# pranoyr/attention-models

Measured on AMD Instinct MI355X. Metric: ViTVQGAN 256px train-step images/sec, higher is better.
Workload: dtype f32; 1 GPU; BASELINE.json configs[2]: ViTVQGAN dim=256 patch=8 img=256 depth=6+6 h=8 d=64 mlp=2048 (SwiGLU), codebook 8192x32; GAN train step (D phase + G phase, gradient penalty, per_loss_weight=0), Adam, clip 1.0; global_batch=32, batch_per_gpu=32, parallelism=dp1

## Files before the change

### attention-models_amd/amk/lib.py

```python
import ctypes
import os
import re

_HERE = os.path.dirname(os.path.abspath(__file__))
LIB_PATH = os.environ.get("AMK_LIB") or os.path.join(_HERE, "libamk.so")
HEADER_PATH = os.path.normpath(os.path.join(_HERE, "..", "..", "include", "amk.h"))

AMK_OK = 0

_c = ctypes
_P = _c.c_void_p
_I = _c.c_int
_L = _c.c_int64
_F = _c.c_float



class GemmDesc(_c.Structure):
    _fields_ = [("op", _c.c_int32), ("epilogue", _c.c_int32), ("m", _L),
                ("n", _c.c_int32), ("k", _c.c_int32), ("split", _c.c_int32), ("reserved", _c.c_int32),
                ("a", _P), ("a2", _P), ("w", _P), ("w2", _P), ("c", _P), ("c2", _P),
                ("lda", _L), ("lda2", _L), ("ldw", _L), ("ldw2", _L), ("ldc", _L), ("ldc2", _L),
                ("bias", _P), ("bias2", _P), ("resid", _P), ("ldr", _L),
                ("ln_mean", _P), ("ln_rstd", _P), ("ln_gamma", _P), ("ln_beta", _P),
                ("ab", _P), ("ldab", _L), ("gate", _P), ("ldg", _L), ("dbias", _P)]


GEMM_NT, GEMM_NN, GEMM_TN = 0, 1, 2
EPI_BIAS, EPI_RESID, EPI_SWIGLU, EPI_SWIGLU_BWD = 0, 1, 2, 3

SIGNATURES = {
    "amk_version": (_I, []),
    "amk_arch": (_c.c_char_p, []),
    "amk_last_error": (_c.c_char_p, []),
    "amk_attn_fwd": (_I, [_P] * 7 + [_I] * 5 + [_L] * 12 + [_F, _P]),
    "amk_attn_scores_bytes": (_L, [_I, _I, _I, _I]),
    "amk_attn_fwd_keep": (_I, [_P] * 8 + [_I] * 5 + [_L] * 12 + [_F, _P]),
    "amk_attn_fwd_x6_ws_bytes": (_L, [_I, _I, _I]),
    "amk_attn_fwd_x6": (_I, [_P] * 8 + [_I] * 5 + [_L] * 12 + [_F, _P]),
    "amk_attn_bwd_ws_floats": (_L, [_I, _I, _I, _I, _I]),
    "amk_attn_bwd": (_I, [_P] * 12 + [_I] * 5 + [_L] * 24 + [_F, _I, _P]),
    "amk_attn_bwd_kept": (_I, [_P] * 13 + [_I] * 5 + [_L] * 24 + [_F, _I, _P]),
    "amk_vq_num_partials": (_L, [_L]),
    "amk_vq_lookup_fwd": (_I, [_P, _P, _L, _I, _I, _I] + [_P] * 9 + [_P]),
    "amk_vq_lookup_bwd": (_I, [_P] * 7 + [_F, _L, _I, _I, _P, _P, _P]),
    "amk_vq_lookup_bwd_rows": (_I, [_P] * 7 + [_F, _L, _I, _I, _P, _P, _P]),
    "amk_vq_padded_codes": (_I, [_I, _I]),
    "amk_vq_gather": (_I, [_P, _P, _L, _I, _I, _P, _P, _P]),
    "amk_agent_num_chunks": (_I, [_I]),
    "amk_agent_ws_floats": (_L, [_I, _I, _I, _I, _I]),
    "amk_agent_attn_fwd": (_I, [_P] * 10 + [_I] * 5 + [_L] * 12 + [_F, _P]),
    "amk_agent_attn_bwd": (_I, [_P] * 14 + [_I] * 5 + [_L] * 21 + [_F, _P]),
    "amk_agent_conv_grad_reduce": (_I, [_P, _P, _L, _I, _P, _P, _P]),
    "amk_rowsum_num_partials": (_I, [_L]),
    "amk_add_layernorm_fwd": (_I, [_P, _P, _P, _P, _L, _I, _F, _P, _P, _P, _P, _P]),
    "amk_add_layernorm_bwd": (_I, [_P, _P, _P, _P, _P, _P, _L, _I, _P, _P, _P]),
    "amk_colsum": (_I, [_P, _L, _I, _P, _P]),
    "amk_swiglu_fwd": (_I, [_P, _L, _I, _P, _P]),
    "amk_swiglu_bwd": (_I, [_P, _P, _L, _I, _P, _P]),
    "amk_geglu_fwd": (_I, [_P, _L, _I, _P, _P]),
    "amk_geglu_bwd": (_I, [_P, _P, _L, _I, _P, _P]),
    "amk_opt_num_partials": (_I, []),
    "amk_sumsq_partials": (_I, [_P, _L, _P, _P]),
    "amk_adam_flat_step": (_I, [_P] * 4 + [_L, _P, _P, _P, _I] + [_F] * 6 + [_I, _P, _P]),
    "amk_adam_flat_step_shadow": (_I, [_P] * 4 + [_L, _P, _P, _P, _I] + [_F] * 6 + [_I, _P, _P, _P]),
    "amk_gemm_x6_planes_bytes": (_L, [_I, _I]),
    "amk_gemm_x6_split": (_I, [_P, _L, _I, _I, _P, _P]),
    "amk_gemm_x6_nt": (_I, [_P, _L, _P, _P, _P, _L, _I, _I, _I, _P]),
    "amk_gemm_f32_ws_bytes": (_L, [_c.POINTER(GemmDesc)]),
    "amk_gemm_f32": (_I, [_c.POINTER(GemmDesc), _P, _L, _P]),
    "amk_row_stats": (_I, [_P, _L, _I, _F, _P, _P, _P]),
    "amk_attn_bf16_fwd": (_I, [_P] * 7 + [_I] * 5 + [_L] * 12 + [_F, _P]),
    "amk_attn_bf16_bwd_ws_floats": (_L, [_I, _I, _I, _I]),
    "amk_attn_bf16_bwd": (_I, [_P] * 12 + [_I] * 5 + [_L] * 24 + [_F, _P]),
    "amk_swiglu_bf16_fwd": (_I, [_P, _L, _I, _P, _P]),
    "amk_swiglu_bf16_bwd": (_I, [_P, _P, _L, _I, _P, _P]),
    "amk_add_layernorm_mixed_fwd": (_I, [_P, _I, _P, _P, _P, _L, _I, _F, _P, _P, _P, _P, _P]),
    "amk_add_layernorm_mixed_bwd": (_I, [_P, _I, _P, _P, _P, _P, _P, _L, _I, _P, _P, _P, _P]),
    "amk_gemm_bf16": (_I, [_I, _I, _P, _L, _P, _L, _P, _P, _L, _P, _L, _L, _I, _I, _P]),
    "amk_gemm_bf16_swiglu_bwd": (_I, [_P, _L, _P, _L, _P, _L, _P, _L, _L, _I, _I, _P]),
    "amk_gemm_tn_bf16_ws_bytes": (_L, [_L, _I, _I]),
    "amk_gemm_tn_bf16": (_I, [_P, _L, _P, _L, _P, _L, _P, _L, _I, _I, _P, _L, _P]),
    "amk_sample_step": (_I, [_P, _P, _F, _P, _c.c_uint64, _c.c_uint64, _F, _L, _I, _I, _P, _F, _P, _P, _P]),
    "amk_moe_route_ws_ints": (_L, [_L, _I, _I]),
    "amk_moe_route": (_I, [_P, _L, _I, _I] + [_P] * 8),
    "amk_grouped_gemm_nt": (_I, [_P, _L, _I, _P, _P, _P, _P, _L, _I, _I, _I, _P, _P]),
    "amk_grouped_gemm_nn": (_I, [_P, _L, _I, _P, _P, _P, _P, _L, _I, _I, _I, _P, _P]),
    "amk_grouped_gemm_nt_acc": (_I, [_P, _L, _I, _P, _P, _P, _P, _L, _I, _I, _I, _P, _I, _P]),
    "amk_grouped_gemm_nn_acc": (_I, [_P, _L, _I, _P, _P, _P, _P, _L, _I, _I, _I, _P, _I, _P]),
    "amk_grouped_gemm_wgrad": (_I, [_P, _L, _I, _P, _L, _I, _P, _P, _P, _L, _I, _I, _I, _P, _P, _P]),
    "amk_moe_combine": (_I, [_P, _P, _P, _L, _I, _I, _I, _P, _P]),
    "amk_moe_expert_sums": (_I, [_P, _L, _I, _P, _P, _L, _I, _I, _I, _P, _P]),
    "amk_moe_topk": (_I, [_P, _L, _I, _I, _P, _P, _P]),
    "amk_moe_route_distinct": (_I, [_P, _L, _I, _I, _P, _P, _P, _P]),
    "amk_moe_combine_rows": (_I, [_P, _P, _P, _L, _I, _I, _I, _I, _I, _P, _P]),
    "amk_moe_gate_grad_rows": (_I, [_P, _P, _P, _P, _L, _I, _I, _I, _I, _I, _P, _P]),
    "amk_moe_gate_grad": (_I, [_P, _P, _P, _P, _L, _I, _I, _I, _I, _P, _P]),
}

_lib = None


def declared_symbols(header_path=HEADER_PATH):
    text = open(header_path).read()
    text = re.sub(r"/\*.*?\*/", "", text, flags=re.S)
    return sorted(set(re.findall(r"\b(amk_[a-z0-9_]+)\s*\(", text)))


def load():
    global _lib
    if _lib is not None:
        return _lib
    if not os.path.exists(LIB_PATH):
        raise RuntimeError(
            f"{LIB_PATH} is missing: build it with `python -c 'import __graft_entry__ as g; g.build()'` "
            "(hipcc --offload-arch=gfx950). amk has no CPU or eager fallback."
        )
    lib = ctypes.CDLL(LIB_PATH)
    for name, (res, args) in SIGNATURES.items():
        fn = getattr(lib, name)
        fn.restype = res
        fn.argtypes = args
    arch = lib.amk_arch().decode()
    if arch != "gfx950":
        raise RuntimeError(f"libamk.so was built for {arch}, expected gfx950")
    _lib = lib
    return lib


def check(rc, what):
    if rc != AMK_OK:
        msg = load().amk_last_error().decode()
        raise RuntimeError(f"{what} failed with code {rc}: {msg}")
```

### attention-models_amd/amk/models/discriminator.py

```python
import contextlib

import torch
import torch.nn as nn
import torch.nn.functional as F
from torch.nn.grad import conv2d_input, conv2d_weight

_INPUT_GRAD_ONLY = False


@contextlib.contextmanager
def input_grad_only():
    global _INPUT_GRAD_ONLY
    old, _INPUT_GRAD_ONLY = _INPUT_GRAD_ONLY, True
    try:
        yield
    finally:
        _INPUT_GRAD_ONLY = old


class _ConvDataGrad(torch.autograd.Function):

    @staticmethod
    def forward(ctx, gy, weight, x_shape, stride, padding):
        ctx.save_for_backward(gy, weight)
        ctx.cfg = (stride, padding)
        return conv2d_input(x_shape, weight, gy, stride=stride, padding=padding)

    @staticmethod
    def backward(ctx, ggx):
        gy, weight = ctx.saved_tensors
        stride, padding = ctx.cfg
        ggx = ggx.contiguous()
        ggy = F.conv2d(ggx, weight, None, stride, padding) if ctx.needs_input_grad[0] else None
        gw = conv2d_weight(ggx, weight.shape, gy, stride=stride, padding=padding) if ctx.needs_input_grad[1] else None
        return ggy, gw, None, None, None


class _Conv(torch.autograd.Function):
    @staticmethod
    def forward(ctx, x, weight, bias, stride, padding):
        ctx.save_for_backward(x, weight)
        ctx.cfg = (stride, padding, bias is not None)
        return F.conv2d(x, weight, bias, stride, padding)

    @staticmethod
    def backward(ctx, gy):
        x, weight = ctx.saved_tensors
        stride, padding, has_bias = ctx.cfg
        gy = gy.contiguous()
        gx = _ConvDataGrad.apply(gy, weight, x.shape, stride, padding) if ctx.needs_input_grad[0] else None
        gw = gb = None
        if not _INPUT_GRAD_ONLY:
            if ctx.needs_input_grad[1]:
                gw = conv2d_weight(x, weight.shape, gy, stride=stride, padding=padding)
            if has_bias and ctx.needs_input_grad[2]:
                gb = gy.sum((0, 2, 3))
        return gx, gw, gb, None, None


class Conv2d(nn.Conv2d):

    def forward(self, x):
        if self.groups != 1 or self.dilation != (1, 1) or self.padding_mode != "zeros" or isinstance(self.padding, str):
            return super().forward(x)
        if torch.is_autocast_enabled():
            if self.in_channels < 8 and x.is_cuda:
                with torch.autocast("cuda", enabled=False):
                    return _Conv.apply(x.float(), self.weight, self.bias, self.stride, self.padding)
            return super().forward(x)
        return _Conv.apply(x, self.weight, self.bias, self.stride, self.padding)


class NLayerDiscriminator(nn.Module):
    def __init__(self, input_nc=3, ndf=64, n_layers=3):
        super().__init__()
        widths = [ndf * min(2 ** i, 8) for i in range(n_layers + 1)]
        layers = [Conv2d(input_nc, widths[0], 4, stride=2, padding=1), nn.LeakyReLU(0.2, True)]
        for i in range(1, n_layers + 1):
            stride = 2 if i < n_layers else 1
            layers += [
                Conv2d(widths[i - 1], widths[i], 4, stride=stride, padding=1, bias=False),
                nn.BatchNorm2d(widths[i]),
                nn.LeakyReLU(0.2, True),
            ]
        layers.append(Conv2d(widths[-1], 1, 4, stride=1, padding=1))
        self.model = nn.Sequential(*layers)

    def forward(self, x):
        return self.model(x)
```

### attention-models_amd/amk/ops.py

```python
import ctypes
import os
import weakref

import torch
from torch.autograd.function import once_differentiable

from . import lib as _lib

_NULL = ctypes.c_void_p(0)


def _ptr(t):
    return ctypes.c_void_p(t.data_ptr()) if t is not None else _NULL


def _stream():
    return ctypes.c_void_p(torch.cuda.current_stream().cuda_stream)


KERNEL_EVENTS = None


class _timed:

# ... 1256 lines not shown
        dwa = dwb = None
        if ctx.needs_input_grad[1] or ctx.needs_input_grad[2]:
            (ar, av), (br, bv) = _claim(ctx.params[0]), _claim(ctx.params[1])
            dwa, dwb, _ = dense.gemm_tn(da2, x2, y2=db2, out=av, out2=bv)
            if av is not None:
                ar.wrote(ctx.params[0])
                dwa = None
            if bv is not None:
                br.wrote(ctx.params[1])
                dwb = None
        return dx, dwa, dwb


class _SwiGLUFFN(torch.autograd.Function):

    @staticmethod
    def forward(ctx, x, w12, b12, w3, b3):
        from . import dense

        x2 = x.reshape(-1, x.shape[-1])
        need = any(ctx.needs_input_grad)
        gate, ab = dense.gemm_nt_swiglu(x2, w12, b12, keep_ab=need)
        out = dense.gemm_nt(gate, w3, b3)
        if need:
            ctx.save_for_backward(x2, w12, w3, ab, gate)
        ctx.x_shape = x.shape
        ctx.has_bias = (b12 is not None, b3 is not None)
        ctx.params = (w12, b12, w3, b3)
        return out.view(*x.shape[:-1], w3.shape[0])

    @staticmethod
    @once_differentiable
    def backward(ctx, dout):
        from . import dense

        x2, w12, w3, ab, gate = ctx.saved_tensors
        d2 = dout.reshape(-1, dout.shape[-1])
        d_ab = dense.gemm_nn(d2, w3, swiglu_ab=ab)
        dw3, db3 = _tn_into(dense.gemm_tn, d2, gate, ctx.params[2], ctx.params[3] if ctx.has_bias[1] else None)
        dx = _nn_plain(d_ab, w12).view(ctx.x_shape) if ctx.needs_input_grad[0] else None
        dw12, db12 = _tn_into(dense.gemm_tn, d_ab, x2, ctx.params[0], ctx.params[1] if ctx.has_bias[0] else None)
        return dx, dw12, db12, dw3, db3


MIXED_WGRAD = os.environ.get("AMK_MIXED_WGRAD", "1") == "1"


def _w16(t):
    if t is None:
        return None
    shadow = getattr(t, "_amk_bf16", None)
    if shadow is not None and t._version == t._amk_bf16_version:
        return shadow
    return t.to(torch.bfloat16)


class _LinearMixed(torch.autograd.Function):

    @staticmethod
    def forward(ctx, x, weight, bias):
        x16, w16 = x.to(torch.bfloat16), _w16(weight)
        ctx.save_for_backward(x16, w16)
        ctx.has_bias, ctx.x_dtype = bias is not None, x.dtype
        ctx.params = (weight, bias)
        return torch.nn.functional.linear(x16, w16, _w16(bias))

    @staticmethod
    @once_differentiable
    def backward(ctx, dy):
        from . import dense

        x16, w16 = ctx.saved_tensors
        dy2 = dy.reshape(-1, dy.shape[-1])
        dx = dy2.mm(w16).view(x16.shape).to(ctx.x_dtype) if ctx.needs_input_grad[0] else None
        dw, db = _tn_into(dense.gemm_tn_bf16, dy2, x16.reshape(-1, x16.shape[-1]), ctx.params[0], ctx.params[1])
        return dx, dw, db


def _mixed_linear_ok(x, weight):
    return (MIXED_WGRAD and x.is_cuda and torch.get_autocast_dtype("cuda") == torch.bfloat16 and torch.is_grad_enabled()
            and weight.requires_grad and weight.dtype == torch.float32 and x.dtype in (torch.float32, torch.bfloat16)
            and weight.shape[0] % 8 == 0 and weight.shape[1] % 8 == 0 and x.numel() > 0)


def linear(x, weight, bias=None):
    if torch.is_autocast_enabled():
        if _mixed_linear_ok(x, weight):
            return _LinearMixed.apply(x, weight, bias)
        return torch.nn.functional.linear(x, weight, bias)
    if GEMM_MODE == "bf16x6" and _x6_ok(x, weight):
        return _LinearX6.apply(x, weight, bias)
    if _dense_ok(x, weight):
        return _DenseLinear.apply(x, weight, bias)
    if bias is None:
        return torch.nn.functional.linear(x, weight)
    return _BiasLinear.apply(x, weight, bias)


def linear2(x, wa, wb):
    if GEMM_MODE != "bf16x6" and _dense_ok(x, wa, wb) and wa.shape[0] % 128 == 0:
        return _DenseLinear2.apply(x, wa, wb)
    return linear(x, wa), linear(x, wb)


class _SwiGLUFFNMixed(torch.autograd.Function):

    @staticmethod
    def forward(ctx, x, w12, b12, w3, b3):
        from . import dense

        x16 = x.to(torch.bfloat16).reshape(-1, x.shape[-1])
        w12h, w3h = _w16(w12), _w16(w3)
        g, ab = dense.gemm_nt_swiglu_bf16(x16, w12h, b12)
        y = torch.nn.functional.linear(g, w3h, _w16(b3))
        ctx.save_for_backward(x16, ab, g, w12h, w3h)
        ctx.x_shape, ctx.x_dtype, ctx.bias = x.shape, x.dtype, (b12 is not None, b3 is not None)
        ctx.params = (w12, b12, w3, b3)
        return y.view(*x.shape[:-1], w3.shape[0])

    @staticmethod
    @once_differentiable
    def backward(ctx, dy):
        from . import dense

        x16, ab, g, w12h, w3h = ctx.saved_tensors
        dy2 = dy.reshape(-1, dy.shape[-1])
        dw3, db3 = _tn_into(dense.gemm_tn_bf16, dy2, g, ctx.params[2], ctx.params[3])
        dab = dense.gemm_nn_swiglu_bwd_bf16(dy2, w3h, ab)
        dw12, db12 = _tn_into(dense.gemm_tn_bf16, dab, x16, ctx.params[0], ctx.params[1])
        dx = dab.mm(w12h).view(ctx.x_shape).to(ctx.x_dtype) if ctx.needs_input_grad[0] else None
        return dx, dw12, db12, dw3, db3


def swiglu_ffn(x, w12, b12, w3, b3):
    if torch.is_autocast_enabled() and w12.shape[0] % 16 == 0 and w12.shape[0] >= 1024:
        if _mixed_linear_ok(x, w12) and _mixed_linear_ok(x, w3) and w3.requires_grad:
            with torch.autocast("cuda", enabled=False):
                return _SwiGLUFFNMixed.apply(x, w12, b12, w3, b3)
        no_grad = not torch.is_grad_enabled() or not any(
            t is not None and t.requires_grad for t in (x, w12, b12, w3, b3))
        if (MIXED_WGRAD and no_grad and x.is_cuda and torch.get_autocast_dtype("cuda") == torch.bfloat16
                and w12.dtype == torch.float32 and x.dtype in (torch.float32, torch.bfloat16) and w12.shape[1] % 8 == 0 and x.numel()):
            from . import dense

            g, _ = dense.gemm_nt_swiglu_bf16(x.to(torch.bfloat16).reshape(-1, x.shape[-1]), _w16(w12), b12, keep_ab=False)
            return torch.nn.functional.linear(g, _w16(w3), _w16(b3)).view(*x.shape[:-1], w3.shape[0])
    if GEMM_MODE != "bf16x6" and _dense_ok(x, w12) and w3.shape[1] % 4 == 0 and w3.shape[0] % 4 == 0 and w3.is_contiguous():
        return _SwiGLUFFN.apply(x, w12, b12, w3, b3)
    ab = linear(x, w12, b12)
    if ab.shape[-1] % 8 == 0:
        return linear(swiglu(ab), w3, b3)
    a, b = ab.chunk(2, dim=-1)
    return linear(torch.nn.functional.silu(a) * b, w3, b3)
```

### include/amk.h

```cpp
#ifndef AMK_H_
#define AMK_H_

#include <stdint.h>

#ifdef __cplusplus
extern "C" {
#endif

#define AMK_VERSION 140

enum {
  AMK_OK = 0,
  AMK_EINVAL = -1,
  AMK_EUNSUPPORTED = -2,
  AMK_ELAUNCH = -3
};

int amk_version(void);
const char* amk_arch(void);
const char* amk_last_error(void);

int amk_attn_fwd(const float* q, const float* k, const float* v, float* o, float* stats,
                 const uint8_t* key_mask, const uint8_t* causal_mask,
                 int B, int H, int I, int J, int D,
// ... 56 lines not shown
                      int64_t q_sb, int64_t q_st, int64_t q_sh,
                      int64_t k_sb, int64_t k_st, int64_t k_sh,
                      int64_t v_sb, int64_t v_st, int64_t v_sh,
                      int64_t o_sb, int64_t o_st, int64_t o_sh,
                      int64_t do_sb, int64_t do_st, int64_t do_sh,
                      int64_t dq_sb, int64_t dq_st, int64_t dq_sh,
                      int64_t dk_sb, int64_t dk_st, int64_t dk_sh,
                      int64_t dv_sb, int64_t dv_st, int64_t dv_sh,
                      float scale, int stages, void* stream);

int64_t amk_vq_num_partials(int64_t N);
int amk_vq_padded_codes(int K, int nsplit);
int amk_vq_lookup_fwd(const float* z, const float* codebook, int64_t N, int K, int C, int nsplit,
                      float* en_ws, float* ee_ws, float* pmin_ws, int32_t* pidx_ws,
                      int64_t* idx, float* out, float* zq, float* zn, float* sqerr_partial,
                      void* stream);

int amk_vq_lookup_bwd(const float* z, const float* codebook, const float* zn, const float* zq,
                      const int64_t* idx, const float* g_out, const float* g_loss, float beta,
                      int64_t N, int K, int C, float* dz, float* dcodebook, void* stream);

int amk_vq_lookup_bwd_rows(const float* z, const float* codebook, const float* zn, const float* zq,
                           const int64_t* idx, const float* g_out, const float* g_loss, float beta,
                           int64_t N, int K, int C, float* dz, float* ge_rows, void* stream);

int amk_vq_gather(const int64_t* idx, const float* codebook, int64_t N, int K, int C,
                  float* out, int32_t* bad_count, void* stream);


int64_t amk_moe_route_ws_ints(int64_t U, int E, int k);
int amk_moe_route(const float* logits, int64_t U, int E, int k,
                  int64_t* ids, float* gate, int32_t* counts, int32_t* rank, int32_t* blockhist,
                  int32_t* offsets, int32_t* perm, void* stream);

int amk_grouped_gemm_nt(const float* A, int64_t lda, int a_div, const float* W, const float* bias,
                        const int32_t* offsets, const int32_t* perm, int64_t P, int E, int N, int Kd,
                        float* Y, void* stream);

int amk_grouped_gemm_nn(const float* A, int64_t lda, int a_div, const float* W, const float* scale,
                        const int32_t* offsets, const int32_t* perm, int64_t P, int E, int N, int Kd,
                        float* Y, void* stream);

int amk_grouped_gemm_nt_acc(const float* A, int64_t lda, int a_div, const float* W, const float* bias,
                            const int32_t* offsets, const int32_t* perm, int64_t P, int E, int N, int Kd,
                            float* Y, int y_div, void* stream);
int amk_grouped_gemm_nn_acc(const float* A, int64_t lda, int a_div, const float* W, const float* scale,
                            const int32_t* offsets, const int32_t* perm, int64_t P, int E, int N, int Kd,
                            float* Y, int y_div, void* stream);

int amk_grouped_gemm_wgrad(const float* G, int64_t ldg, int g_div, const float* X, int64_t ldx, int x_div,
                           const float* scale, const int32_t* offsets, const int32_t* perm,
                           int64_t P, int E, int N, int Kd, float* dW, float* dbias, void* stream);

int amk_moe_combine(const float* Y, const int64_t* ids, const float* scale, int64_t G, int outer, int k,
                    int N, float* out, void* stream);

int amk_moe_topk(const float* logits, int64_t U, int E, int k, int64_t* ids, float* gate, void* stream);

int amk_moe_route_distinct(const int64_t* ids, int64_t G, int fan, int E, uint64_t* mask,
                           int32_t* offsets, int32_t* perm, void* stream);

int amk_moe_combine_rows(const float* Y, const int64_t* ids, const float* scale, int64_t G, int outer, int k,
                         int N, int v_div, int E, float* out, void* stream);
int amk_moe_gate_grad_rows(const float* d_out, const float* Y, const int64_t* ids, const float* gate,
                           int64_t P, int k, int E, int N, int g_div, int v_div, float* dlogits, void* stream);

int amk_moe_expert_sums(const float* A, int64_t lda, int a_div, const int64_t* ids, const float* scale,
                        int64_t G, int fan, int E, int d, float* Z, void* stream);

int amk_moe_gate_grad(const float* d_out, const float* Y, const int64_t* ids, const float* gate,
                      int64_t P, int k, int E, int N, int g_div, float* dlogits, void* stream);

int amk_agent_num_chunks(int T);
int64_t amk_agent_ws_floats(int B, int H, int T, int P, int backward);

int amk_agent_attn_fwd(const float* q, const float* k, const float* v, const float* conv_w, const float* conv_b,
                       float* o, float* agents, float* vagent, float* stats1, float* ws,
                       int B, int H, int T, int D, int P,
                       int64_t q_sb, int64_t q_st, int64_t q_sh, int64_t k_sb, int64_t k_st, int64_t k_sh,
                       int64_t v_sb, int64_t v_st, int64_t v_sh, int64_t o_sb, int64_t o_st, int64_t o_sh,
                       float scale, void* stream);

int amk_agent_attn_bwd(const float* q, const float* k, const float* v, const float* conv_w, const float* d_o,
                       const float* agents, const float* vagent, const float* stats1,
                       float* dq, float* dk, float* dv, float* ws, float* dconvw_part, float* dconvb_part,
                       int B, int H, int T, int D, int P,
                       int64_t q_sb, int64_t q_st, int64_t q_sh, int64_t k_sb, int64_t k_st, int64_t k_sh,
                       int64_t v_sb, int64_t v_st, int64_t v_sh, int64_t do_sb, int64_t do_st, int64_t do_sh,
                       int64_t dq_sb, int64_t dq_st, int64_t dq_sh, int64_t dk_sb, int64_t dk_st, int64_t dk_sh,
                       int64_t dv_sb, int64_t dv_st, int64_t dv_sh, float scale, void* stream);

int amk_agent_conv_grad_reduce(const float* dconvw_part, const float* dconvb_part, int64_t rows, int D,
                               float* dconvw, float* dconvb, void* stream);

int amk_rowsum_num_partials(int64_t M);
int amk_add_layernorm_fwd(const float* x, const float* res, const float* gamma, const float* beta,
                          int64_t M, int D, float eps, float* h, float* y, float* mean, float* rstd, void* stream);
int amk_add_layernorm_bwd(const float* dy, const float* h, const float* dh_in, const float* gamma,
                          const float* mean, const float* rstd, int64_t M, int D, float* dh, float* dgb_part,
                          void* stream);
int amk_colsum(const float* x, int64_t M, int N, float* part, void* stream);

int amk_swiglu_fwd(const float* ab, int64_t M, int H, float* out, void* stream);
int amk_swiglu_bwd(const float* ab, const float* d_out, int64_t M, int H, float* d_ab, void* stream);

int amk_geglu_fwd(const float* ab, int64_t M, int H, float* out, void* stream);
int amk_geglu_bwd(const float* ab, const float* d_out, int64_t M, int H, float* d_ab, void* stream);

int amk_opt_num_partials(void);
int amk_sumsq_partials(const float* x, int64_t n, float* partials, void* stream);
int amk_adam_flat_step(float* param, float* grad, float* exp_avg, float* exp_avg_sq, int64_t n,
                       const int32_t* seg_param, const float* param_tab,
                       const float* partials, int n_partials,
                       float max_norm, float lr, float beta1, float beta2, float eps, float weight_decay,
                       int decoupled, float* norm_out, void* stream);
int amk_adam_flat_step_shadow(float* param, float* grad, float* exp_avg, float* exp_avg_sq, int64_t n,
                              const int32_t* seg_param, const float* param_tab,
                              const float* partials, int n_partials,
                              float max_norm, float lr, float beta1, float beta2, float eps, float weight_decay,
                              int decoupled, float* norm_out, void* param_bf16, void* stream);

int amk_sample_step(const float* logits, const float* null_logits, float cfg_scale,
                    const float* gumbel, uint64_t seed, uint64_t offset, float tau,
                    int64_t R, int V, int keep, const uint8_t* mask, float unmasked_score,
                    int64_t* ids, float* scores, void* stream);

int64_t amk_gemm_x6_planes_bytes(int N, int K);
int amk_gemm_x6_split(const float* W, int64_t ldw, int N, int K, void* planes, void* stream);
int amk_gemm_x6_nt(const float* A, int64_t lda, const void* w_planes, const float* bias,
                   float* C, int64_t ldc, int M, int N, int K, void* stream);

enum { AMK_GEMM_NT = 0, AMK_GEMM_NN = 1, AMK_GEMM_TN = 2 };
enum { AMK_EPI_BIAS = 0, AMK_EPI_RESID = 1, AMK_EPI_SWIGLU = 2, AMK_EPI_SWIGLU_BWD = 3 };
typedef struct amk_gemm_desc {
  int32_t op, epilogue;
  int64_t m;
  int32_t n, k, split, reserved;
  const float *a, *a2, *w, *w2;
  float *c, *c2;
  int64_t lda, lda2, ldw, ldw2, ldc, ldc2;
  const float *bias, *bias2, *resid;
  int64_t ldr;
  const float *ln_mean, *ln_rstd, *ln_gamma, *ln_beta;
  const float* ab;
  int64_t ldab;
  float* gate;
  int64_t ldg;
  float* dbias;
} amk_gemm_desc;
int64_t amk_gemm_f32_ws_bytes(const amk_gemm_desc* d);
int amk_gemm_f32(const amk_gemm_desc* d, void* workspace, int64_t ws_bytes, void* stream);
int amk_row_stats(const float* x, int64_t M, int D, float eps, float* mean, float* rstd, void* stream);

int amk_attn_bf16_fwd(const void* q, const void* k, const void* v, void* o, float* stats,
                      const uint8_t* key_mask, const uint8_t* causal_mask,
                      int B, int H, int I, int J, int D,
                      int64_t q_sb, int64_t q_st, int64_t q_sh, int64_t k_sb, int64_t k_st, int64_t k_sh,
                      int64_t v_sb, int64_t v_st, int64_t v_sh, int64_t o_sb, int64_t o_st, int64_t o_sh,
                      float scale, void* stream);
int64_t amk_attn_bf16_bwd_ws_floats(int B, int H, int I, int J);
int amk_attn_bf16_bwd(const void* q, const void* k, const void* v, const void* o, const float* stats, const void* d_o,
                      void* dq, void* dk, void* dv, float* ws,
                      const uint8_t* key_mask, const uint8_t* causal_mask,
                      int B, int H, int I, int J, int D,
                      int64_t q_sb, int64_t q_st, int64_t q_sh, int64_t k_sb, int64_t k_st, int64_t k_sh,
                      int64_t v_sb, int64_t v_st, int64_t v_sh, int64_t o_sb, int64_t o_st, int64_t o_sh,
                      int64_t do_sb, int64_t do_st, int64_t do_sh, int64_t dq_sb, int64_t dq_st, int64_t dq_sh,
                      int64_t dk_sb, int64_t dk_st, int64_t dk_sh, int64_t dv_sb, int64_t dv_st, int64_t dv_sh,
                      float scale, void* stream);

int amk_swiglu_bf16_fwd(const void* ab, int64_t M, int H, void* out, void* stream);
int amk_swiglu_bf16_bwd(const void* ab, const void* d_out, int64_t M, int H, void* d_ab, void* stream);
int amk_add_layernorm_mixed_fwd(const void* x, int x_is_bf16, const float* res, const float* gamma, const float* beta,
                                int64_t M, int D, float eps, float* h, void* y_bf16, float* mean, float* rstd, void* stream);
int amk_add_layernorm_mixed_bwd(const void* dy, int dy_is_bf16, const float* h, const float* dh_in, const float* gamma,
                                const float* mean, const float* rstd, int64_t M, int D, float* dh, void* dh_bf16,
                                float* dgb_part, void* stream);

int64_t amk_gemm_tn_bf16_ws_bytes(int64_t M, int N, int K);
int amk_gemm_tn_bf16(const void* y, int64_t ldy, const void* x, int64_t ldx, float* c, int64_t ldc, float* dbias,
                     int64_t M, int N, int K, void* workspace, int64_t ws_bytes, void* stream);

int amk_gemm_bf16(int op, int epi, const void* a, int64_t lda, const void* w, int64_t ldw, const float* bias,
                  void* c, int64_t ldc, void* g, int64_t ldg, int64_t M, int N, int K, void* stream);

int amk_gemm_bf16_swiglu_bwd(const void* dy, int64_t lddy, const void* w3, int64_t ldw, const void* ab, int64_t ldab,
                             void* dab, int64_t lddab, int64_t M, int H, int K, void* stream);

#ifdef __cplusplus
}
#endif
#endif
```

Before: 296.1 images/s.

## Add custom f32 conv kernels for discriminator single-output and small-input convs

Adds HIP kernels for 4x4 pad-1 convolutions, routed from the discriminator's conv autograd functions. The cases covered are the final Cout=1 layer (forward, data grad, and weight grad with a fused bias grad) and the first layer with Cin<=4 (forward only). These replace MIOpen calls that are likely inefficient for such thin shapes, including those in the gradient-penalty double-backward path. The cost is new code paths with split-reduction workspaces and fallbacks to the library for all other shapes.

```diff
diff --git a/attention-models_amd/amk/lib.py b/attention-models_amd/amk/lib.py
--- a/attention-models_amd/amk/lib.py
+++ b/attention-models_amd/amk/lib.py
@@ -26,6 +26,12 @@
                 ("ab", _P), ("ldab", _L), ("gate", _P), ("ldg", _L), ("dbias", _P)]
 
 
+class ConvDesc(_c.Structure):
+    _fields_ = [(f, _c.c_int32) for f in ("n", "c", "h", "w", "cout", "kh", "kw", "stride", "pad", "reserved")] + [
+        (f, _P) for f in ("x", "weight", "bias", "gy", "y", "gx", "gw", "gb")]
+
+
+CONV_FWD, CONV_DGRAD, CONV_WGRAD = 0, 1, 2
 GEMM_NT, GEMM_NN, GEMM_TN = 0, 1, 2
 EPI_BIAS, EPI_RESID, EPI_SWIGLU, EPI_SWIGLU_BWD = 0, 1, 2, 3
 
@@ -70,6 +76,10 @@
     "amk_gemm_f32_ws_bytes": (_L, [_c.POINTER(GemmDesc)]),
     "amk_gemm_f32": (_I, [_c.POINTER(GemmDesc), _P, _L, _P]),
     "amk_row_stats": (_I, [_P, _L, _I, _F, _P, _P, _P]),
+    "amk_conv_f32_ws_bytes": (_L, [_c.POINTER(ConvDesc), _I]),
+    "amk_conv_f32_fwd": (_I, [_c.POINTER(ConvDesc), _P, _L, _P]),
+    "amk_conv_f32_dgrad": (_I, [_c.POINTER(ConvDesc), _P, _L, _P]),
+    "amk_conv_f32_wgrad": (_I, [_c.POINTER(ConvDesc), _P, _L, _P]),
     "amk_attn_bf16_fwd": (_I, [_P] * 7 + [_I] * 5 + [_L] * 12 + [_F, _P]),
     "amk_attn_bf16_bwd_ws_floats": (_L, [_I, _I, _I, _I]),
     "amk_attn_bf16_bwd": (_I, [_P] * 12 + [_I] * 5 + [_L] * 24 + [_F, _P]),
diff --git a/attention-models_amd/amk/models/discriminator.py b/attention-models_amd/amk/models/discriminator.py
--- a/attention-models_amd/amk/models/discriminator.py
+++ b/attention-models_amd/amk/models/discriminator.py
@@ -2,8 +2,8 @@
 
 import torch
 import torch.nn as nn
-import torch.nn.functional as F
-from torch.nn.grad import conv2d_input, conv2d_weight
+
+from .. import ops
 
 _INPUT_GRAD_ONLY = False
 
@@ -24,15 +24,15 @@
     def forward(ctx, gy, weight, x_shape, stride, padding):
         ctx.save_for_backward(gy, weight)
         ctx.cfg = (stride, padding)
-        return conv2d_input(x_shape, weight, gy, stride=stride, padding=padding)
+        return ops.conv2d_dgrad(x_shape, weight, gy, stride, padding)
 
     @staticmethod
     def backward(ctx, ggx):
         gy, weight = ctx.saved_tensors
         stride, padding = ctx.cfg
         ggx = ggx.contiguous()
-        ggy = F.conv2d(ggx, weight, None, stride, padding) if ctx.needs_input_grad[0] else None
-        gw = conv2d_weight(ggx, weight.shape, gy, stride=stride, padding=padding) if ctx.needs_input_grad[1] else None
+        ggy = ops.conv2d_fwd(ggx, weight, None, stride, padding) if ctx.needs_input_grad[0] else None
+        gw = ops.conv2d_wgrad(ggx, weight.shape, gy, stride, padding)[0] if ctx.needs_input_grad[1] else None
         return ggy, gw, None, None, None
 
 
@@ -41,7 +41,7 @@
     def forward(ctx, x, weight, bias, stride, padding):
         ctx.save_for_backward(x, weight)
         ctx.cfg = (stride, padding, bias is not None)
-        return F.conv2d(x, weight, bias, stride, padding)
+        return ops.conv2d_fwd(x, weight, bias, stride, padding)
 
     @staticmethod
     def backward(ctx, gy):
@@ -51,9 +51,10 @@
         gx = _ConvDataGrad.apply(gy, weight, x.shape, stride, padding) if ctx.needs_input_grad[0] else None
         gw = gb = None
         if not _INPUT_GRAD_ONLY:
+            want_gb = has_bias and ctx.needs_input_grad[2]
             if ctx.needs_input_grad[1]:
-                gw = conv2d_weight(x, weight.shape, gy, stride=stride, padding=padding)
-            if has_bias and ctx.needs_input_grad[2]:
+                gw, gb = ops.conv2d_wgrad(x, weight.shape, gy, stride, padding, bias_grad=want_gb)
+            elif want_gb:
                 gb = gy.sum((0, 2, 3))
         return gx, gw, gb, None, None
 
diff --git a/attention-models_amd/amk/ops.py b/attention-models_amd/amk/ops.py
--- a/attention-models_amd/amk/ops.py
+++ b/attention-models_amd/amk/ops.py
@@ -1432,3 +1432,96 @@
         return linear(swiglu(ab), w3, b3)
     a, b = ab.chunk(2, dim=-1)
     return linear(torch.nn.functional.silu(a) * b, w3, b3)
+
+
+CONV_MODE = os.environ.get("AMK_CONV", "auto")
+
+CONV_AUTO = {("out1", "fwd"), ("out1", "dgrad"), ("out1", "wgrad"), ("in4", "fwd")}
+
+
+def _conv_class(n, c, h, w, cout, weight_hw, stride, padding, direction):
+    if tuple(weight_hw) != (4, 4) or tuple(padding) != (1, 1) or stride[0] != stride[1] or stride[0] not in (1, 2):
+        return None
+    if h + 2 < 4 or w + 2 < 4:
+        return None
+    if cout == 1 and h * w <= 1024:
+        return "out1"
+    if c <= 4 and direction == "fwd":
+        return "in4"
+    return None
+
+
+def _conv_route(direction, x_shape, weight_shape, stride, padding, *tensors):
+    if CONV_MODE == "lib" or torch.is_autocast_enabled():
+        return False
+    for t in tensors:
+        if t is not None and (not t.is_cuda or t.dtype != torch.float32 or not t.is_contiguous()):
+            return False
+    n, c, h, w = x_shape
+    if n == 0:
+        return False
+    cls = _conv_class(n, c, h, w, weight_shape[0], weight_shape[2:], stride, padding, direction)
+    if cls is None:
+        return False
+    return CONV_MODE == "amk" or (cls, direction) in CONV_AUTO
+
+
+def _conv_desc(x_shape, weight_shape, stride):
+    n, c, h, w = x_shape
+    return _lib.ConvDesc(n=n, c=c, h=h, w=w, cout=weight_shape[0], kh=weight_shape[2], kw=weight_shape[3],
+                         stride=stride[0], pad=1)
+
+
+def _conv_run(fn, d, direction, device):
+    L = _lib.load()
+    nbytes = L.amk_conv_f32_ws_bytes(ctypes.byref(d), direction)
+    ws = torch.empty((max(nbytes, 4) + 3) // 4, device=device, dtype=torch.float32)
+    _lib.check(getattr(L, fn)(ctypes.byref(d), _ptr(ws), ws.numel() * 4, _stream()), fn)
+
+
+def _out_hw(h, w, stride):
+    return (h + 2 - 4) // stride[0] + 1, (w + 2 - 4) // stride[0] + 1
+
+
+def conv2d_fwd(x, weight, bias, stride, padding):
+    stride, padding = _pair(stride), _pair(padding)
+    if not _conv_route("fwd", x.shape, weight.shape, stride, padding, x, weight, bias) or x.shape[1] != weight.shape[1]:
+        return torch.nn.functional.conv2d(x, weight, bias, stride, padding)
+    n, _, h, w = x.shape
+    oh, ow = _out_hw(h, w, stride)
+    y = torch.empty((n, weight.shape[0], oh, ow), device=x.device, dtype=torch.float32)
+    d = _conv_desc(x.shape, weight.shape, stride)
+    d.x, d.weight, d.bias, d.y = _ptr(x), _ptr(weight), _ptr(bias), _ptr(y)
+    _conv_run("amk_conv_f32_fwd", d, _lib.CONV_FWD, x.device)
+    return y
+
+
+def conv2d_dgrad(x_shape, weight, gy, stride, padding):
+    stride, padding = _pair(stride), _pair(padding)
+    x_shape = tuple(x_shape)
+    if (not _conv_route("dgrad", x_shape, weight.shape, stride, padding, weight, gy)
+            or tuple(gy.shape[2:]) != _out_hw(x_shape[2], x_shape[3], stride)):
+        return torch.nn.grad.conv2d_input(x_shape, weight, gy, stride=stride, padding=padding)
+    gx = torch.empty(x_shape, device=gy.device, dtype=torch.float32)
+    d = _conv_desc(x_shape, weight.shape, stride)
+    d.gy, d.weight, d.gx = _ptr(gy), _ptr(weight), _ptr(gx)
+    _conv_run("amk_conv_f32_dgrad", d, _lib.CONV_DGRAD, gy.device)
+    return gx
+
+
+def conv2d_wgrad(x, weight_shape, gy, stride, padding, bias_grad=False):
+    stride, padding = _pair(stride), _pair(padding)
+    weight_shape = tuple(weight_shape)
+    if not _conv_route("wgrad", x.shape, weight_shape, stride, padding, x, gy) or x.shape[1] != weight_shape[1]:
+        gw = torch.nn.grad.conv2d_weight(x, weight_shape, gy, stride=stride, padding=padding)
+        return gw, (gy.sum((0, 2, 3)) if bias_grad else None)
+    gw = torch.empty(weight_shape, device=x.device, dtype=torch.float32)
+    gb = torch.empty((weight_shape[0],), device=x.device, dtype=torch.float32) if bias_grad else None
+    d = _conv_desc(x.shape, weight_shape, stride)
+    d.x, d.gy, d.gw, d.gb = _ptr(x), _ptr(gy), _ptr(gw), _ptr(gb)
+    _conv_run("amk_conv_f32_wgrad", d, _lib.CONV_WGRAD, x.device)
+    return gw, gb
+
+
+def _pair(v):
+    return tuple(v) if isinstance(v, (tuple, list)) else (v, v)
diff --git a/attention-models_amd/csrc/conv_f32.hip b/attention-models_amd/csrc/conv_f32.hip
--- /dev/null
+++ b/attention-models_amd/csrc/conv_f32.hip
@@ -0,0 +1,334 @@
+#include "amk_common.h"
+
+namespace {
+
+constexpr int CV_THREADS = 256;
+constexpr int CV_PPT = 4;
+constexpr int CV_MAX_PLANE = CV_THREADS * CV_PPT;
+constexpr int CV_TAPS = 16;
+constexpr int CV_FWD_GROUP = 32;
+constexpr int CV_DGRAD_GROUP = 32;
+constexpr int CV_WGRAD_GROUP = 8;
+constexpr int CV_WGRAD_SPLIT = 8;
+
+struct Geom {
+  int n, c, h, w, oh, ow, stride, pad;
+};
+
+__host__ __device__ __forceinline__ int cdiv(int a, int b) { return (a + b - 1) / b; }
+
+__device__ __forceinline__ int tap_src(const Geom& g, int ih, int iw, int kh, int kw) {
+  const int th = ih + g.pad - kh, tw = iw + g.pad - kw;
+  if (th < 0 || tw < 0) return -1;
+  if (g.stride == 2 && ((th | tw) & 1)) return -1;
+  const int oh = g.stride == 2 ? th >> 1 : th, ow = g.stride == 2 ? tw >> 1 : tw;
+  if (oh >= g.oh || ow >= g.ow) return -1;
+  return oh * g.ow + ow;
+}
+
+__global__ __launch_bounds__(CV_THREADS) void conv_c1_fwd_partial(const float* __restrict__ x, const float* __restrict__ w,
+                                                                  float* __restrict__ part, Geom g) {
+  __shared__ float z[CV_TAPS * CV_MAX_PLANE];
+  const int t = threadIdx.x, grp = blockIdx.x, n = blockIdx.y, ngrp = gridDim.x;
+  const int hw = g.h * g.w, ohw = g.oh * g.ow;
+  const int c0 = grp * CV_FWD_GROUP, c1 = min(g.c, c0 + CV_FWD_GROUP);
+  const float* xn = x + (int64_t)n * g.c * hw;
+  float acc[CV_PPT][CV_TAPS];
+#pragma unroll
+  for (int j = 0; j < CV_PPT; ++j)
+#pragma unroll
+    for (int k = 0; k < CV_TAPS; ++k) acc[j][k] = 0.f;
+#pragma unroll 2
+  for (int c = c0; c < c1; ++c) {
+    const float* xc = xn + (int64_t)c * hw;
+    const float* wc = w + c * CV_TAPS;
+    float v[CV_PPT];
+#pragma unroll
+    for (int j = 0; j < CV_PPT; ++j) {
+      const int p = t + j * CV_THREADS;
+      v[j] = p < hw ? xc[p] : 0.f;
+    }
+#pragma unroll
+    for (int k = 0; k < CV_TAPS; ++k) {
+      const float wk = wc[k];
+#pragma unroll
+      for (int j = 0; j < CV_PPT; ++j) acc[j][k] = fmaf(v[j], wk, acc[j][k]);
+    }
+  }
+#pragma unroll
+  for (int j = 0; j < CV_PPT; ++j)
+#pragma unroll
+    for (int k = 0; k < CV_TAPS; ++k) z[k * CV_MAX_PLANE + t + j * CV_THREADS] = acc[j][k];
+  __syncthreads();
+  float* pn = part + ((int64_t)n * ngrp + grp) * ohw;
+  for (int q = t; q < ohw; q += CV_THREADS) {
+    const int oh = q / g.ow, ow = q - oh * g.ow;
+    float s = 0.f;
+#pragma unroll
+    for (int kh = 0; kh < 4; ++kh) {
+      const int ih = oh * g.stride - g.pad + kh;
+#pragma unroll
+      for (int kw = 0; kw < 4; ++kw) {
+        const int iw = ow * g.stride - g.pad + kw;
+        if (ih >= 0 && ih < g.h && iw >= 0 && iw < g.w) s += z[(kh * 4 + kw) * CV_MAX_PLANE + ih * g.w + iw];
+      }
+    }
+    pn[q] = s;
+  }
+}
+
+__global__ __launch_bounds__(CV_THREADS) void conv_c1_fwd_reduce(const float* __restrict__ part, const float* __restrict__ bias,
+                                                                 float* __restrict__ y, int n_img, int ngrp, int ohw) {
+  const int64_t i = (int64_t)blockIdx.x * CV_THREADS + threadIdx.x;
+  if (i >= (int64_t)n_img * ohw) return;
+  const int n = (int)(i / ohw), q = (int)(i - (int64_t)n * ohw);
+  const float* pn = part + (int64_t)n * ngrp * ohw + q;
+  float s = 0.f;
+  for (int gi = 0; gi < ngrp; ++gi) s += pn[(int64_t)gi * ohw];
+  y[i] = bias ? s + bias[0] : s;
+}
+
+__global__ __launch_bounds__(CV_THREADS) void conv_c1_dgrad(const float* __restrict__ gy, const float* __restrict__ w,
+                                                            float* __restrict__ gx, Geom g) {
+  const int t = threadIdx.x, n = blockIdx.y;
+  const int hw = g.h * g.w;
+  const int c0 = blockIdx.x * CV_DGRAD_GROUP, c1 = min(g.c, c0 + CV_DGRAD_GROUP);
+  const float* gyn = gy + (int64_t)n * g.oh * g.ow;
+  float tv[CV_PPT][CV_TAPS];
+#pragma unroll
+  for (int j = 0; j < CV_PPT; ++j) {
+    const int p = t + j * CV_THREADS;
+    const int ih = p / g.w, iw = p - ih * g.w;
+#pragma unroll
+    for (int k = 0; k < CV_TAPS; ++k) {
+      const int src = p < hw ? tap_src(g, ih, iw, k >> 2, k & 3) : -1;
+      tv[j][k] = src >= 0 ? gyn[src] : 0.f;
+    }
+  }
+  float* gxn = gx + (int64_t)n * g.c * hw;
+#pragma unroll 2
+  for (int c = c0; c < c1; ++c) {
+    const float* wc = w + c * CV_TAPS;
+    float* gxc = gxn + (int64_t)c * hw;
+    float s[CV_PPT];
+#pragma unroll
+    for (int j = 0; j < CV_PPT; ++j) s[j] = 0.f;
+#pragma unroll
+    for (int k = 0; k < CV_TAPS; ++k) {
+      const float wk = wc[k];
+#pragma unroll
+      for (int j = 0; j < CV_PPT; ++j) s[j] = fmaf(tv[j][k], wk, s[j]);
+    }
+#pragma unroll
+    for (int j = 0; j < CV_PPT; ++j) {
+      const int p = t + j * CV_THREADS;
+      if (p < hw) gxc[p] = s[j];
+    }
+  }
+}
+
+__global__ __launch_bounds__(CV_THREADS) void conv_c1_wgrad_partial(const float* __restrict__ x, const float* __restrict__ gy,
+                                                                    float* __restrict__ part, Geom g) {
+  __shared__ float red[CV_THREADS / AMK_WAVE][CV_WGRAD_GROUP * CV_TAPS];
+  const int t = threadIdx.x, sl = blockIdx.y, nsplit = gridDim.y;
+  const int hw = g.h * g.w, ohw = g.oh * g.ow;
+  const int c0 = blockIdx.x * CV_WGRAD_GROUP, nc = min(g.c - c0, CV_WGRAD_GROUP);
+  float acc[CV_WGRAD_GROUP][CV_TAPS];
+#pragma unroll
+  for (int c = 0; c < CV_WGRAD_GROUP; ++c)
+#pragma unroll
+    for (int k = 0; k < CV_TAPS; ++k) acc[c][k] = 0.f;
+  for (int n = sl; n < g.n; n += nsplit) {
+    const float* gyn = gy + (int64_t)n * ohw;
+    const float* xn = x + ((int64_t)n * g.c + c0) * hw;
+#pragma unroll 1
+    for (int j = 0; j < CV_PPT; ++j) {
+      const int p = t + j * CV_THREADS;
+      if (p >= hw) break;
+      const int ih = p / g.w, iw = p - ih * g.w;
+      float xv[CV_WGRAD_GROUP];
+#pragma unroll
+      for (int c = 0; c < CV_WGRAD_GROUP; ++c) xv[c] = c < nc ? xn[(int64_t)c * hw + p] : 0.f;
+#pragma unroll
+      for (int k = 0; k < CV_TAPS; ++k) {
+        const int src = tap_src(g, ih, iw, k >> 2, k & 3);
+        const float tk = src >= 0 ? gyn[src] : 0.f;
+#pragma unroll
+        for (int c = 0; c < CV_WGRAD_GROUP; ++c) acc[c][k] = fmaf(xv[c], tk, acc[c][k]);
+      }
+    }
+  }
+  const int lane = t & (AMK_WAVE - 1), wave = t / AMK_WAVE;
+#pragma unroll
+  for (int c = 0; c < CV_WGRAD_GROUP; ++c)
+#pragma unroll
+    for (int k = 0; k < CV_TAPS; ++k) {
+      float v = acc[c][k];
+#pragma unroll
+      for (int o = AMK_WAVE / 2; o > 0; o >>= 1) v += __shfl_xor(v, o);
+      if (lane == 0) red[wave][c * CV_TAPS + k] = v;
+    }
+  __syncthreads();
+  if (t < nc * CV_TAPS) {
+    float s = red[0][t];
+#pragma unroll
+    for (int wv = 1; wv < CV_THREADS / AMK_WAVE; ++wv) s += red[wv][t];
+    part[(int64_t)sl * g.c * CV_TAPS + c0 * CV_TAPS + t] = s;
+  }
+}
+
+__global__ __launch_bounds__(CV_THREADS) void conv_c1_wgrad_reduce(const float* __restrict__ part, const float* __restrict__ gy,
+                                                                   float* __restrict__ gw, float* __restrict__ gb, int nw,
+                                                                   int nsplit, int64_t ny) {
+  const int t = threadIdx.x;
+  if (blockIdx.x * CV_THREADS < nw) {
+    const int i = blockIdx.x * CV_THREADS + t;
+    if (i >= nw) return;
+    float s = 0.f;
+    for (int sl = 0; sl < nsplit; ++sl) s += part[(int64_t)sl * nw + i];
+    gw[i] = s;
+    return;
+  }
+  __shared__ float red[CV_THREADS / AMK_WAVE];
+  float s = 0.f;
+  for (int64_t i = t; i < ny; i += CV_THREADS) s += gy[i];
+#pragma unroll
+  for (int o = AMK_WAVE / 2; o > 0; o >>= 1) s += __shfl_xor(s, o);
+  if ((t & (AMK_WAVE - 1)) == 0) red[t / AMK_WAVE] = s;
+  __syncthreads();
+  if (t == 0) {
+    float b = red[0];
+    for (int wv = 1; wv < CV_THREADS / AMK_WAVE; ++wv) b += red[wv];
+    gb[0] = b;
+  }
+}
+
+template <int CIN>
+__global__ __launch_bounds__(CV_THREADS) void conv_cin_fwd(const float* __restrict__ x, const float* __restrict__ w,
+                                                           const float* __restrict__ bias, float* __restrict__ y,
+                                                           int cout, Geom g) {
+  const int n = blockIdx.y, ohw = g.oh * g.ow, hw = g.h * g.w;
+  const int q = blockIdx.x * CV_THREADS + threadIdx.x;
+  if (q >= ohw) return;
+  const int oh = q / g.ow, ow = q - oh * g.ow;
+  const float* xn = x + (int64_t)n * CIN * hw;
+  float xv[CIN * CV_TAPS];
+#pragma unroll
+  for (int ci = 0; ci < CIN; ++ci)
+#pragma unroll
+    for (int kh = 0; kh < 4; ++kh) {
+      const int ih = oh * g.stride - g.pad + kh;
+#pragma unroll
+      for (int kw = 0; kw < 4; ++kw) {
+        const int iw = ow * g.stride - g.pad + kw;
+        const bool in = ih >= 0 && ih < g.h && iw >= 0 && iw < g.w;
+        xv[ci * CV_TAPS + kh * 4 + kw] = in ? xn[(int64_t)ci * hw + ih * g.w + iw] : 0.f;
+      }
+    }
+  float* yn = y + (int64_t)n * cout * ohw + q;
+#pragma unroll 2
+  for (int co = 0; co < cout; ++co) {
+    const float* wc = w + co * CIN * CV_TAPS;
+    float s = 0.f;
+#pragma unroll
+    for (int i = 0; i < CIN * CV_TAPS; ++i) s = fmaf(xv[i], wc[i], s);
+    yn[(int64_t)co * ohw] = bias ? s + bias[co] : s;
+  }
+}
+
+int check_desc(const amk_conv_desc* d, const char* what, Geom* g) {
+  AMK_CHECK_ARG(d, "%s: null descriptor", what);
+  AMK_CHECK_ARG(d->n > 0 && d->c > 0 && d->h > 0 && d->w > 0 && d->cout > 0, "%s: non-positive size", what);
+  AMK_CHECK_SUPPORTED(d->kh == 4 && d->kw == 4, "%s: only 4 x 4 kernels are built", what);
+  AMK_CHECK_SUPPORTED(d->pad == 1 && (d->stride == 1 || d->stride == 2), "%s: only pad 1, stride 1 or 2 are built", what);
+  g->n = d->n, g->c = d->c, g->h = d->h, g->w = d->w, g->stride = d->stride, g->pad = d->pad;
+  g->oh = (d->h + 2 * d->pad - 4) / d->stride + 1;
+  g->ow = (d->w + 2 * d->pad - 4) / d->stride + 1;
+  AMK_CHECK_SUPPORTED(g->oh > 0 && g->ow > 0, "%s: image smaller than the kernel", what);
+  AMK_CHECK_SUPPORTED((int64_t)d->n * d->c * d->h * d->w < (int64_t)1 << 31 &&
+                          (int64_t)d->n * d->cout * g->oh * g->ow < (int64_t)1 << 31,
+                      "%s: tensor too large", what);
+  return AMK_OK;
+}
+
+bool one_out(const amk_conv_desc* d) { return d->cout == 1 && d->h * d->w <= CV_MAX_PLANE; }
+
+int wgrad_split(const amk_conv_desc* d) { return d->n < CV_WGRAD_SPLIT ? d->n : CV_WGRAD_SPLIT; }
+
+}
+
+extern "C" int64_t amk_conv_f32_ws_bytes(const amk_conv_desc* d, int dir) {
+  Geom g;
+  if (check_desc(d, "amk_conv_f32_ws_bytes", &g) != AMK_OK || !one_out(d)) return 0;
+  if (dir == AMK_CONV_FWD) return (int64_t)d->n * cdiv(d->c, CV_FWD_GROUP) * g.oh * g.ow * (int64_t)sizeof(float);
+  if (dir == AMK_CONV_WGRAD) return (int64_t)wgrad_split(d) * d->c * CV_TAPS * (int64_t)sizeof(float);
+  return 0;
+}
+
+extern "C" int amk_conv_f32_fwd(const amk_conv_desc* d, void* workspace, int64_t ws_bytes, void* stream) {
+  Geom g;
+  int rc = check_desc(d, "amk_conv_f32_fwd", &g);
+  if (rc != AMK_OK) return rc;
+  AMK_CHECK_ARG(d->x && d->weight && d->y, "amk_conv_f32_fwd: null operand");
+  hipStream_t st = static_cast<hipStream_t>(stream);
+  const float* x = static_cast<const float*>(d->x);
+  const float* w = static_cast<const float*>(d->weight);
+  const float* b = static_cast<const float*>(d->bias);
+  float* y = static_cast<float*>(d->y);
+  const int ohw = g.oh * g.ow;
+  if (one_out(d)) {
+    const int ngrp = cdiv(d->c, CV_FWD_GROUP);
+    AMK_CHECK_ARG(workspace && ws_bytes >= amk_conv_f32_ws_bytes(d, AMK_CONV_FWD), "amk_conv_f32_fwd: workspace too small");
+    float* part = static_cast<float*>(workspace);
+    hipLaunchKernelGGL(conv_c1_fwd_partial, dim3(ngrp, d->n), dim3(CV_THREADS), 0, st, x, w, part, g);
+    AMK_CHECK_LAUNCH("amk_conv_f32_fwd(partial)");
+    hipLaunchKernelGGL(conv_c1_fwd_reduce, dim3(cdiv(d->n * ohw, CV_THREADS)), dim3(CV_THREADS), 0, st, part, b, y,
+                       d->n, ngrp, ohw);
+    AMK_CHECK_LAUNCH("amk_conv_f32_fwd(reduce)");
+    return AMK_OK;
+  }
+  const dim3 grid(cdiv(ohw, CV_THREADS), d->n);
+  switch (d->c) {
+    case 1: hipLaunchKernelGGL(conv_cin_fwd<1>, grid, dim3(CV_THREADS), 0, st, x, w, b, y, d->cout, g); break;
+    case 2: hipLaunchKernelGGL(conv_cin_fwd<2>, grid, dim3(CV_THREADS), 0, st, x, w, b, y, d->cout, g); break;
+    case 3: hipLaunchKernelGGL(conv_cin_fwd<3>, grid, dim3(CV_THREADS), 0, st, x, w, b, y, d->cout, g); break;
+    case 4: hipLaunchKernelGGL(conv_cin_fwd<4>, grid, dim3(CV_THREADS), 0, st, x, w, b, y, d->cout, g); break;
+    default: AMK_CHECK_SUPPORTED(false, "amk_conv_f32_fwd: built for Cout == 1 (H * W <= %d) or Cin <= 4", CV_MAX_PLANE);
+  }
+  AMK_CHECK_LAUNCH("amk_conv_f32_fwd");
+  return AMK_OK;
+}
+
+extern "C" int amk_conv_f32_dgrad(const amk_conv_desc* d, void* workspace, int64_t ws_bytes, void* stream) {
+  (void)workspace, (void)ws_bytes;
+  Geom g;
+  int rc = check_desc(d, "amk_conv_f32_dgrad", &g);
+  if (rc != AMK_OK) return rc;
+  AMK_CHECK_SUPPORTED(one_out(d), "amk_conv_f32_dgrad: built for Cout == 1, H * W <= %d", CV_MAX_PLANE);
+  AMK_CHECK_ARG(d->gy && d->weight && d->gx, "amk_conv_f32_dgrad: null operand");
+  hipLaunchKernelGGL(conv_c1_dgrad, dim3(cdiv(d->c, CV_DGRAD_GROUP), d->n), dim3(CV_THREADS), 0,
+                     static_cast<hipStream_t>(stream), static_cast<const float*>(d->gy), static_cast<const float*>(d->weight),
+                     static_cast<float*>(d->gx), g);
+  AMK_CHECK_LAUNCH("amk_conv_f32_dgrad");
+  return AMK_OK;
+}
+
+extern "C" int amk_conv_f32_wgrad(const amk_conv_desc* d, void* workspace, int64_t ws_bytes, void* stream) {
+  Geom g;
+  int rc = check_desc(d, "amk_conv_f32_wgrad", &g);
+  if (rc != AMK_OK) return rc;
+  AMK_CHECK_SUPPORTED(one_out(d), "amk_conv_f32_wgrad: built for Cout == 1, H * W <= %d", CV_MAX_PLANE);
+  AMK_CHECK_ARG(d->x && d->gy && d->gw, "amk_conv_f32_wgrad: null operand");
+  AMK_CHECK_ARG(workspace && ws_bytes >= amk_conv_f32_ws_bytes(d, AMK_CONV_WGRAD), "amk_conv_f32_wgrad: workspace too small");
+  hipStream_t st = static_cast<hipStream_t>(stream);
+  const int nsplit = wgrad_split(d), nw = d->c * CV_TAPS;
+  float* part = static_cast<float*>(workspace);
+  hipLaunchKernelGGL(conv_c1_wgrad_partial, dim3(cdiv(d->c, CV_WGRAD_GROUP), nsplit), dim3(CV_THREADS), 0, st,
+                     static_cast<const float*>(d->x), static_cast<const float*>(d->gy), part, g);
+  AMK_CHECK_LAUNCH("amk_conv_f32_wgrad(partial)");
+  const int nblk = cdiv(nw, CV_THREADS) + (d->gb ? 1 : 0);
+  hipLaunchKernelGGL(conv_c1_wgrad_reduce, dim3(nblk), dim3(CV_THREADS), 0, st, part, static_cast<const float*>(d->gy),
+                     static_cast<float*>(d->gw), static_cast<float*>(d->gb), nw, nsplit, (int64_t)d->n * g.oh * g.ow);
+  AMK_CHECK_LAUNCH("amk_conv_f32_wgrad(reduce)");
+  return AMK_OK;
+}
diff --git a/include/amk.h b/include/amk.h
--- a/include/amk.h
+++ b/include/amk.h
@@ -232,6 +232,19 @@
 int amk_gemm_f32(const amk_gemm_desc* d, void* workspace, int64_t ws_bytes, void* stream);
 int amk_row_stats(const float* x, int64_t M, int D, float eps, float* mean, float* rstd, void* stream);
 
+enum { AMK_CONV_FWD = 0, AMK_CONV_DGRAD = 1, AMK_CONV_WGRAD = 2 };
+typedef struct amk_conv_desc {
+  int32_t n, c, h, w;
+  int32_t cout, kh, kw;
+  int32_t stride, pad, reserved;
+  const float *x, *weight, *bias, *gy;
+  float *y, *gx, *gw, *gb;
+} amk_conv_desc;
+int64_t amk_conv_f32_ws_bytes(const amk_conv_desc* d, int dir);
+int amk_conv_f32_fwd(const amk_conv_desc* d, void* workspace, int64_t ws_bytes, void* stream);
+int amk_conv_f32_dgrad(const amk_conv_desc* d, void* workspace, int64_t ws_bytes, void* stream);
+int amk_conv_f32_wgrad(const amk_conv_desc* d, void* workspace, int64_t ws_bytes, void* stream);
+
 int amk_attn_bf16_fwd(const void* q, const void* k, const void* v, void* o, float* stats,
                       const uint8_t* key_mask, const uint8_t* causal_mask,
                       int B, int H, int I, int J, int D,
```

Result: faster. 299.9 images/s (median of 6 runs) (+1.3%).
